# neonbjb/tortoise-tts

Hardware: NVIDIA H100
Metric: audio-seconds/sec at preset='standard' (higher is better)
Workload: dtype bf16 tensor-core operands, fp32 accumulate/residual/norm/softmax/scheduler

## Files before the change

tortoise_tts_b200/csrc/flash_attn.cu:

```cuda
#include <type_traits>

#include "common.cuh"
#include "ttb_internal.h"

namespace ttb {

constexpr int FA_BM = 128;
constexpr int FA_BN = 64;
constexpr int FA_CONSUMERS = 256;
constexpr int FA_PRODUCER_WARP = 8;
constexpr int FA_THREADS = FA_CONSUMERS + 32;
constexpr int FA_STAGES = 2;

struct FaSmem {
  static constexpr int Q_BYTES = FA_BM * 64 * 2;
  static constexpr int K_BYTES = FA_BN * 64 * 2;
  static constexpr int V_BYTES = FA_BN * 64 * 2;
  static constexpr int Q_OFF = 0;
  static constexpr int KV_OFF = Q_BYTES;
  static constexpr int BIAS_OFF = KV_OFF + FA_STAGES * (K_BYTES + V_BYTES);
  static constexpr int BAR_OFF = BIAS_OFF + 192 * 4;
  static constexpr int TOTAL = BAR_OFF + 16 * 8 + 1024;
};

__global__ void __launch_bounds__(FA_THREADS, 2)
flash_attn_tc_kernel(const __grid_constant__ CUtensorMap map_q, const __grid_constant__ CUtensorMap map_k,
                     const __grid_constant__ CUtensorMap map_v, TtbAttnArgs a) {
  extern __shared__ uint8_t smem_raw[];
  uint8_t* smem = reinterpret_cast<uint8_t*>((reinterpret_cast<uintptr_t>(smem_raw) + 1023) & ~uintptr_t(1023));
  uint64_t* bars = reinterpret_cast<uint64_t*>(smem + FaSmem::BAR_OFF);
  uint64_t* q_full = bars + 0;
  uint64_t* kv_full = bars + 1;
  uint64_t* kv_empty = bars + 1 + FA_STAGES;
  float* sbias = reinterpret_cast<float*>(smem + FaSmem::BIAS_OFF);

  const int warp = threadIdx.x >> 5, lane = threadIdx.x & 31;
  const int q0 = blockIdx.x * FA_BM, h = blockIdx.y, seq = blockIdx.z;
  const int Tq = a.T;
  const int T = a.Tk > 0 ? a.Tk : a.T;
  const int kv_end = a.causal ? min(T, q0 + FA_BM) : T;
  const int kc0 = a.kv_headmajor ? 0 : a.k_off + h * 64;
  const int vc0 = a.kv_headmajor ? 0 : a.v_off + h * 64;
  const int kvc2 = a.kv_headmajor ? h : seq;
  const int ntiles = (kv_end + FA_BN - 1) / FA_BN;

  if (warp == FA_PRODUCER_WARP && lane == 0) {
    tma_prefetch_desc(&map_q);
    tma_prefetch_desc(&map_k);
    tma_prefetch_desc(&map_v);
    mbar_init(q_full, 1);
    for (int s = 0; s < FA_STAGES; ++s) { mbar_init(&kv_full[s], 1); mbar_init(&kv_empty[s], 2); }
    fence_barrier_init();
  }
  __syncthreads();
  pdl_wait();

  if (warp == FA_PRODUCER_WARP) {
    if (lane == 0) {
      mbar_arrive_expect_tx(q_full, FaSmem::Q_BYTES);
      tma_load_3d(smem + FaSmem::Q_OFF, &map_q, q_full, h * 64, q0, seq);
      int stage = 0; uint32_t phase = 0;
      for (int j = 0; j < ntiles; ++j) {
        mbar_wait(&kv_empty[stage], phase ^ 1);
        uint8_t* sk = smem + FaSmem::KV_OFF + stage * (FaSmem::K_BYTES + FaSmem::V_BYTES);
        uint8_t* sv = sk + FaSmem::K_BYTES;
        mbar_arrive_expect_tx(&kv_full[stage], FaSmem::K_BYTES + FaSmem::V_BYTES);
        tma_load_3d(sk, &map_k, &kv_full[stage], kc0, j * FA_BN, kvc2);
        tma_load_3d(sv, &map_v, &kv_full[stage], vc0, j * FA_BN, kvc2);
        if (++stage == FA_STAGES) { stage = 0; phase ^= 1; }
      }
    }
    __syncwarp();
  } else {
    const int wg = warp >> 2;
    const int g = lane >> 2, t = lane & 3;
    const int row0 = wg * 64 + (warp & 3) * 16 + g;
    const float sl2 = a.scale * 1.4426950408889634f;
    const float* bias_h = a.bias ? a.bias + (long long)h * (2 * T - 1) + (T - 1) : nullptr;
    float m[2] = {-INFINITY, -INFINITY}, l[2] = {0.f, 0.f};
    float o[32];
#pragma unroll
    for (int i = 0; i < 32; ++i) o[i] = 0.f;
    const uint32_t sq = smem_u32(smem + FaSmem::Q_OFF) + wg * (64 * 128);
    mbar_wait(q_full, 0);
    int stage = 0; uint32_t phase = 0;
    for (int j = 0; j < ntiles; ++j) {
      const int k0 = j * FA_BN;
      const bool nomask = (k0 + FA_BN <= T) && (!a.causal || k0 + FA_BN - 1 <= q0);
      bool cbias_ok = (bias_h == nullptr);
      float cb = 0.f;
      if (bias_h && a.bias_sat > 0) {
        if (k0 - q0 + (FA_BN - 1) <= -a.bias_sat) { cbias_ok = true; cb = __ldg(bias_h - (T - 1)) * 1.4426950408889634f; }
        else if (k0 - q0 - (FA_BM - 1) >= a.bias_sat) { cbias_ok = true; cb = __ldg(bias_h + (T - 1)) * 1.4426950408889634f; }
      }
      const bool fast = nomask && cbias_ok;
      if (bias_h && !fast) {
        named_barrier(1, FA_CONSUMERS);
        for (int i = threadIdx.x; i < 191; i += FA_CONSUMERS) {
          const int rel = k0 - q0 - 127 + i;
          sbias[i] = (rel > -T && rel < T) ? __ldg(bias_h + rel) * 1.4426950408889634f : 0.f;
        }
        named_barrier(1, FA_CONSUMERS);
      }
      mbar_wait(&kv_full[stage], phase);
      const uint32_t sk = smem_u32(smem + FaSmem::KV_OFF + stage * (FaSmem::K_BYTES + FaSmem::V_BYTES));
      const uint32_t sv = sk + FaSmem::K_BYTES;
      float s[32];
      wgmma_fence();
#pragma unroll
      for (int k = 0; k < 4; ++k)
        wgmma_m64n64k16_bf16_ss(s, wgmma_desc_kmajor_sw128(sq + k * 32), wgmma_desc_kmajor_sw128(sk + k * 32), k != 0);
      wgmma_commit();
      wgmma_wait<0>();
      float mx[2] = {-INFINITY, -INFINITY};
      if (fast) {
#pragma unroll
        for (int i = 0; i < 32; ++i) mx[(i >> 1) & 1] = fmaxf(mx[(i >> 1) & 1], s[i]);
        mx[0] = fmaf(mx[0], sl2, cb);
        mx[1] = fmaf(mx[1], sl2, cb);
      } else {
#pragma unroll
        for (int i = 0; i < 32; ++i) {
          const int hh = (i >> 1) & 1;
          const int row = row0 + 8 * hh;
          const int c = 8 * (i >> 2) + 2 * t + (i & 1);
          const int klim = min(T - k0, a.causal ? (q0 + row - k0 + 1) : FA_BN);
          float v = s[i] * sl2;
          if (bias_h) v += sbias[c - row + 127];
          v = (c < klim) ? v : -INFINITY;
          s[i] = v;
          mx[hh] = fmaxf(mx[hh], v);
        }
      }
      float corr[2], cm[2];
#pragma unroll
      for (int hh = 0; hh < 2; ++hh) {
        mx[hh] = fmaxf(mx[hh], __shfl_xor_sync(0xffffffffu, mx[hh], 1));
        mx[hh] = fmaxf(mx[hh], __shfl_xor_sync(0xffffffffu, mx[hh], 2));
        const bool grow = mx[hh] > m[hh] + 8.0f;
        const float m_new = grow ? mx[hh] : m[hh];
        corr[hh] = grow ? exp2f(m[hh] - m_new) : 1.0f;
        m[hh] = m_new;
        const float m_use = (m_new == -INFINITY) ? 0.f : m_new;
        cm[hh] = fast ? cb - m_use : -m_use;
      }
      float psum[2] = {0.f, 0.f};
      uint32_t pa[16];
#pragma unroll
      for (int i = 0; i < 32; i += 2) {
        const int hh = (i >> 1) & 1;
        const float p0 = fast ? exp2f(fmaf(s[i], sl2, cm[hh])) : exp2f(s[i] + cm[hh]);
        const float p1 = fast ? exp2f(fmaf(s[i + 1], sl2, cm[hh])) : exp2f(s[i + 1] + cm[hh]);
        psum[hh] += p0 + p1;
        pa[i >> 1] = pack_bf16(p0, p1);
      }
#pragma unroll
      for (int hh = 0; hh < 2; ++hh) l[hh] = l[hh] * corr[hh] + psum[hh];
#pragma unroll
      for (int i = 0; i < 32; ++i) o[i] *= corr[(i >> 1) & 1];
      wgmma_fence();
#pragma unroll
      for (int k = 0; k < 4; ++k)
        wgmma_m64n64k16_bf16_rs<1>(o, pa + 4 * k, wgmma_desc_mnmajor_sw128(sv + k * 2048, 0), 1u);
      wgmma_commit();
      wgmma_wait<0>();
      if ((threadIdx.x & 127) == 0) mbar_arrive(&kv_empty[stage]);
      if (++stage == FA_STAGES) { stage = 0; phase ^= 1; }
    }
#pragma unroll
    for (int hh = 0; hh < 2; ++hh) {
      l[hh] += __shfl_xor_sync(0xffffffffu, l[hh], 1);
      l[hh] += __shfl_xor_sync(0xffffffffu, l[hh], 2);
      const int qi = q0 + row0 + 8 * hh;
      if (qi >= Tq) continue;
      const float inv = 1.0f / l[hh];
      if (a.lse) {
        float* op = a.out_f32 + ((long long)seq * Tq + qi) * a.ldo + h * 64 + 2 * t;
#pragma unroll
        for (int nb = 0; nb < 8; ++nb)
          *reinterpret_cast<float2*>(op + 8 * nb) = make_float2(o[4 * nb + 2 * hh] * inv, o[4 * nb + 2 * hh + 1] * inv);
        if (t == 0) a.lse[((long long)seq * Tq + qi) * a.H + h] = m[hh] + log2f(l[hh]);
      } else {
        __nv_bfloat16* op = reinterpret_cast<__nv_bfloat16*>(a.out) + ((long long)seq * Tq + qi) * a.ldo + h * 64 + 2 * t;
#pragma unroll
        for (int nb = 0; nb < 8; ++nb)
          *reinterpret_cast<uint32_t*>(op + 8 * nb) = pack_bf16(o[4 * nb + 2 * hh] * inv, o[4 * nb + 2 * hh + 1] * inv);
      }
    }
  }
  pdl_launch_dependents();
}

static int g_fa_mode = -1;

bool flash_attention_supported(const TtbAttnArgs& a) {
  if (g_fa_mode < 0) {
    const char* e = getenv("TTB_ATTN_IMPL");
    g_fa_mode = (e && strcmp(e, "simt") == 0) ? 0 : 1;
  }
  if (!g_fa_mode) return false;
  if (a.kv || a.lse) return true;
  return a.T >= 64 && (a.ld % 8) == 0;
}

int flash_attention_launch(const TtbAttnArgs& a, cudaStream_t st) {
  CUtensorMap mq, mk, mv;
  if (get_tensor_map_bf16(&mq, a.qkv, (uint64_t)a.ld, (uint64_t)a.T, (uint64_t)a.nseq, (uint64_t)a.ld,
                          (uint64_t)a.T * a.ld, 64, FA_BM)) return -1;
  if (a.kv_headmajor) {
    if (!a.kv || !a.kv_v || a.Tk <= 0 || a.causal || a.bias) { set_error("flash attention: bad head-major KV arguments"); return -1; }
    if (get_tensor_map_bf16(&mk, a.kv, 64, (uint64_t)a.Tk, (uint64_t)a.H, 64, (uint64_t)a.Tk * 64, 64, FA_BN)) return -1;
    if (get_tensor_map_bf16(&mv, a.kv_v, 64, (uint64_t)a.Tk, (uint64_t)a.H, 64, (uint64_t)a.Tk * 64, 64, FA_BN)) return -1;
  } else {
    if (a.Tk > 0 && a.Tk != a.T) { set_error("flash attention: Tk != T needs the head-major KV form"); return -1; }
    if (get_tensor_map_bf16(&mk, a.qkv, (uint64_t)a.ld, (uint64_t)a.T, (uint64_t)a.nseq, (uint64_t)a.ld,
                            (uint64_t)a.T * a.ld, 64, FA_BN)) return -1;
    mv = mk;
  }
  if (a.lse && !a.out_f32) { set_error("flash attention: lse output needs out_f32"); return -1; }
  static bool attr = false;
  if (!attr) {
    cudaError_t r = cudaFuncSetAttribute(flash_attn_tc_kernel, cudaFuncAttributeMaxDynamicSharedMemorySize, FaSmem::TOTAL);
    if (r != cudaSuccess) return check_cuda(r, "cudaFuncSetAttribute(flash_attn)");
    attr = true;
  }
  dim3 grid((a.T + FA_BM - 1) / FA_BM, a.H, a.nseq);
  const cudaError_t le = launch_pdl(flash_attn_tc_kernel, grid, dim3(FA_THREADS), (size_t)FaSmem::TOTAL, st, mq, mk, mv, a);
  if (le != cudaSuccess) return check_cuda(le, "flash_attn_tc_kernel launch");
  TTB_CHECK_LAUNCH("flash_attn_tc_kernel");
  return 0;
}

}
```

Baseline: 7.400.

## Make flash attention persistent and warp-specialized with overlapped QK and PV wgmma

Result: faster. 7.492 (median of 6 runs) (+1.2%).

```diff
diff --git a/tortoise_tts_b200/csrc/flash_attn.cu b/tortoise_tts_b200/csrc/flash_attn.cu
--- a/tortoise_tts_b200/csrc/flash_attn.cu
+++ b/tortoise_tts_b200/csrc/flash_attn.cu
@@ -7,184 +7,299 @@
 
 constexpr int FA_BM = 128;
 constexpr int FA_BN = 64;
-constexpr int FA_CONSUMERS = 256;
-constexpr int FA_PRODUCER_WARP = 8;
-constexpr int FA_THREADS = FA_CONSUMERS + 32;
-constexpr int FA_STAGES = 2;
+constexpr int FA_THREADS = 384;
+constexpr int FA_STAGES = 4;
+constexpr int FA_TAB = 1024;
+constexpr float FA_L2E = 1.4426950408889634f;
 
 struct FaSmem {
   static constexpr int Q_BYTES = FA_BM * 64 * 2;
   static constexpr int K_BYTES = FA_BN * 64 * 2;
   static constexpr int V_BYTES = FA_BN * 64 * 2;
+  static constexpr int KV_BYTES = K_BYTES + V_BYTES;
   static constexpr int Q_OFF = 0;
-  static constexpr int KV_OFF = Q_BYTES;
-  static constexpr int BIAS_OFF = KV_OFF + FA_STAGES * (K_BYTES + V_BYTES);
-  static constexpr int BAR_OFF = BIAS_OFF + 192 * 4;
+  static constexpr int KV_OFF = 2 * Q_BYTES;
+  static constexpr int BIAS_OFF = KV_OFF + FA_STAGES * KV_BYTES;
+  static constexpr int BAR_OFF = BIAS_OFF + 2 * FA_TAB * 4;
   static constexpr int TOTAL = BAR_OFF + 16 * 8 + 1024;
 };
 
-__global__ void __launch_bounds__(FA_THREADS, 2)
-flash_attn_tc_kernel(const __grid_constant__ CUtensorMap map_q, const __grid_constant__ CUtensorMap map_k,
+template <int N>
+TTB_DEVINL void fa_pin(float* r) {
+#pragma unroll
+  for (int i = 0; i < N; ++i) asm volatile("" : "+f"(r[i])::"memory");
+}
+template <int N>
+TTB_DEVINL void fa_pin(uint32_t* r) {
+#pragma unroll
+  for (int i = 0; i < N; ++i) asm volatile("" : "+r"(r[i])::"memory");
+}
+
+TTB_DEVINL void fa_unit(const TtbAttnArgs& a, int u, int nqb, int& seq, int& h, int& q0) {
+  const int sh = a.H * a.nseq;
+  const int qb = u / sh, r = u - qb * sh;
+  q0 = (a.causal ? nqb - 1 - qb : qb) * FA_BM;
+  seq = r / a.H;
+  h = r - seq * a.H;
+}
+
+__global__ void __launch_bounds__(FA_THREADS, 1)
+flash_attn_ws_kernel(const __grid_constant__ CUtensorMap map_q, const __grid_constant__ CUtensorMap map_k,
                      const __grid_constant__ CUtensorMap map_v, TtbAttnArgs a) {
   extern __shared__ uint8_t smem_raw[];
   uint8_t* smem = reinterpret_cast<uint8_t*>((reinterpret_cast<uintptr_t>(smem_raw) + 1023) & ~uintptr_t(1023));
   uint64_t* bars = reinterpret_cast<uint64_t*>(smem + FaSmem::BAR_OFF);
   uint64_t* q_full = bars + 0;
-  uint64_t* kv_full = bars + 1;
-  uint64_t* kv_empty = bars + 1 + FA_STAGES;
-  float* sbias = reinterpret_cast<float*>(smem + FaSmem::BIAS_OFF);
+  uint64_t* q_empty = bars + 2;
+  uint64_t* kv_full = bars + 4;
+  uint64_t* kv_empty = bars + 4 + FA_STAGES;
 
   const int warp = threadIdx.x >> 5, lane = threadIdx.x & 31;
-  const int q0 = blockIdx.x * FA_BM, h = blockIdx.y, seq = blockIdx.z;
   const int Tq = a.T;
   const int T = a.Tk > 0 ? a.Tk : a.T;
-  const int kv_end = a.causal ? min(T, q0 + FA_BM) : T;
-  const int kc0 = a.kv_headmajor ? 0 : a.k_off + h * 64;
-  const int vc0 = a.kv_headmajor ? 0 : a.v_off + h * 64;
-  const int kvc2 = a.kv_headmajor ? h : seq;
-  const int ntiles = (kv_end + FA_BN - 1) / FA_BN;
-
-  if (warp == FA_PRODUCER_WARP && lane == 0) {
+  const int nqb = (Tq + FA_BM - 1) / FA_BM;
+  const int units = nqb * a.H * a.nseq;
+
+  if (threadIdx.x == 0) {
     tma_prefetch_desc(&map_q);
     tma_prefetch_desc(&map_k);
     tma_prefetch_desc(&map_v);
-    mbar_init(q_full, 1);
+    for (int b = 0; b < 2; ++b) { mbar_init(&q_full[b], 1); mbar_init(&q_empty[b], 8); }
     for (int s = 0; s < FA_STAGES; ++s) { mbar_init(&kv_full[s], 1); mbar_init(&kv_empty[s], 2); }
     fence_barrier_init();
   }
   __syncthreads();
   pdl_wait();
 
-  if (warp == FA_PRODUCER_WARP) {
-    if (lane == 0) {
-      mbar_arrive_expect_tx(q_full, FaSmem::Q_BYTES);
-      tma_load_3d(smem + FaSmem::Q_OFF, &map_q, q_full, h * 64, q0, seq);
+  if (warp < 4) {
+    setmaxnreg_dec<40>();
+    if (threadIdx.x == 0) {
       int stage = 0; uint32_t phase = 0;
-      for (int j = 0; j < ntiles; ++j) {
-        mbar_wait(&kv_empty[stage], phase ^ 1);
-        uint8_t* sk = smem + FaSmem::KV_OFF + stage * (FaSmem::K_BYTES + FaSmem::V_BYTES);
-        uint8_t* sv = sk + FaSmem::K_BYTES;
-        mbar_arrive_expect_tx(&kv_full[stage], FaSmem::K_BYTES + FaSmem::V_BYTES);
-        tma_load_3d(sk, &map_k, &kv_full[stage], kc0, j * FA_BN, kvc2);
-        tma_load_3d(sv, &map_v, &kv_full[stage], vc0, j * FA_BN, kvc2);
-        if (++stage == FA_STAGES) { stage = 0; phase ^= 1; }
+      int it = 0;
+      for (int u = blockIdx.x; u < units; u += gridDim.x, ++it) {
+        int seq, h, q0;
+        fa_unit(a, u, nqb, seq, h, q0);
+        const int kc0 = a.kv_headmajor ? 0 : a.k_off + h * 64;
+        const int vc0 = a.kv_headmajor ? 0 : a.v_off + h * 64;
+        const int kvc2 = a.kv_headmajor ? h : seq;
+        const int kv_end = a.causal ? min(T, q0 + FA_BM) : T;
+        const int ntiles = (kv_end + FA_BN - 1) / FA_BN;
+        const int qbuf = it & 1;
+        mbar_wait(&q_empty[qbuf], ((it >> 1) & 1) ^ 1);
+        mbar_arrive_expect_tx(&q_full[qbuf], FaSmem::Q_BYTES);
+        tma_load_3d(smem + FaSmem::Q_OFF + qbuf * FaSmem::Q_BYTES, &map_q, &q_full[qbuf], h * 64, q0, seq);
+        for (int j = 0; j < ntiles; ++j) {
+          mbar_wait(&kv_empty[stage], phase ^ 1);
+          uint8_t* sk = smem + FaSmem::KV_OFF + stage * FaSmem::KV_BYTES;
+          mbar_arrive_expect_tx(&kv_full[stage], FaSmem::KV_BYTES);
+          tma_load_3d(sk, &map_k, &kv_full[stage], kc0, j * FA_BN, kvc2);
+          tma_load_3d(sk + FaSmem::K_BYTES, &map_v, &kv_full[stage], vc0, j * FA_BN, kvc2);
+          if (++stage == FA_STAGES) { stage = 0; phase ^= 1; }
+        }
       }
     }
     __syncwarp();
   } else {
-    const int wg = warp >> 2;
+    setmaxnreg_inc<232>();
+    const int wg = (warp >> 2) - 1;
+    const int wtid = threadIdx.x & 127;
     const int g = lane >> 2, t = lane & 3;
     const int row0 = wg * 64 + (warp & 3) * 16 + g;
-    const float sl2 = a.scale * 1.4426950408889634f;
-    const float* bias_h = a.bias ? a.bias + (long long)h * (2 * T - 1) + (T - 1) : nullptr;
-    float m[2] = {-INFINITY, -INFINITY}, l[2] = {0.f, 0.f};
-    float o[32];
-#pragma unroll
-    for (int i = 0; i < 32; ++i) o[i] = 0.f;
-    const uint32_t sq = smem_u32(smem + FaSmem::Q_OFF) + wg * (64 * 128);
-    mbar_wait(q_full, 0);
+    const float sl2 = a.scale * FA_L2E;
+    const int bar_tab = 1 + wg;
+    const bool unit_tab = a.bias && a.bias_sat > 0 && 2 * a.bias_sat + 1 <= FA_TAB;
+    float* tab = reinterpret_cast<float*>(smem + FaSmem::BIAS_OFF) + wg * FA_TAB;
     int stage = 0; uint32_t phase = 0;
-    for (int j = 0; j < ntiles; ++j) {
-      const int k0 = j * FA_BN;
-      const bool nomask = (k0 + FA_BN <= T) && (!a.causal || k0 + FA_BN - 1 <= q0);
-      bool cbias_ok = (bias_h == nullptr);
-      float cb = 0.f;
+    int it = 0;
+    for (int u = blockIdx.x; u < units; u += gridDim.x, ++it) {
+      int seq, h, q0;
+      fa_unit(a, u, nqb, seq, h, q0);
+      const int kv_end = a.causal ? min(T, q0 + FA_BM) : T;
+      const int ntiles = (kv_end + FA_BN - 1) / FA_BN;
+      const float* bias_h = a.bias ? a.bias + (long long)h * (2 * T - 1) + (T - 1) : nullptr;
+      float cb_lo = 0.f, cb_hi = 0.f;
       if (bias_h && a.bias_sat > 0) {
-        if (k0 - q0 + (FA_BN - 1) <= -a.bias_sat) { cbias_ok = true; cb = __ldg(bias_h - (T - 1)) * 1.4426950408889634f; }
-        else if (k0 - q0 - (FA_BM - 1) >= a.bias_sat) { cbias_ok = true; cb = __ldg(bias_h + (T - 1)) * 1.4426950408889634f; }
-      }
-      const bool fast = nomask && cbias_ok;
-      if (bias_h && !fast) {
-        named_barrier(1, FA_CONSUMERS);
-        for (int i = threadIdx.x; i < 191; i += FA_CONSUMERS) {
-          const int rel = k0 - q0 - 127 + i;
-          sbias[i] = (rel > -T && rel < T) ? __ldg(bias_h + rel) * 1.4426950408889634f : 0.f;
-        }
-        named_barrier(1, FA_CONSUMERS);
-      }
+        cb_lo = __ldg(bias_h - (T - 1)) * FA_L2E;
+        cb_hi = __ldg(bias_h + (T - 1)) * FA_L2E;
+      }
+      if (unit_tab) {
+        named_barrier(bar_tab, 128);
+        for (int i = wtid; i <= 2 * a.bias_sat; i += 128) {
+          const int rel = i - a.bias_sat;
+          tab[i] = (rel > -T && rel < T) ? __ldg(bias_h + rel) * FA_L2E : 0.f;
+        }
+        named_barrier(bar_tab, 128);
+      }
+      const int qbuf = it & 1;
+      mbar_wait(&q_full[qbuf], (it >> 1) & 1);
+      uint32_t qa[16];
+      {
+        const uint8_t* sq = smem + FaSmem::Q_OFF + qbuf * FaSmem::Q_BYTES;
+        const int r = row0;
+#pragma unroll
+        for (int k = 0; k < 4; ++k) {
+#pragma unroll
+          for (int hi = 0; hi < 2; ++hi) {
+            const int chunk = (2 * k + hi) ^ (r & 7);
+            qa[4 * k + 2 * hi] = *reinterpret_cast<const uint32_t*>(sq + r * 128 + chunk * 16 + 4 * t);
+            qa[4 * k + 2 * hi + 1] = *reinterpret_cast<const uint32_t*>(sq + (r + 8) * 128 + chunk * 16 + 4 * t);
+          }
+        }
+      }
+      __syncwarp();
+      if (lane == 0) mbar_arrive(&q_empty[qbuf]);
+
+      float m[2] = {-INFINITY, -INFINITY}, l[2] = {0.f, 0.f};
+      float o[32], s[32], corr[2];
+      float x[32];
+      uint32_t pa[16];
+#pragma unroll
+      for (int i = 0; i < 32; ++i) o[i] = 0.f;
+
+      auto issue_s = [&](int st) {
+        const uint32_t sk = smem_u32(smem + FaSmem::KV_OFF + st * FaSmem::KV_BYTES);
+#pragma unroll
+        for (int k = 0; k < 4; ++k) wgmma_m64n64k16_bf16_rs<0>(s, qa + 4 * k, wgmma_desc_kmajor_sw128(sk + k * 32), k != 0);
+        wgmma_commit();
+      };
+      auto issue_pv = [&](int st) {
+        const uint32_t sv = smem_u32(smem + FaSmem::KV_OFF + st * FaSmem::KV_BYTES + FaSmem::K_BYTES);
+#pragma unroll
+        for (int k = 0; k < 4; ++k) wgmma_m64n64k16_bf16_rs<1>(o, pa + 4 * k, wgmma_desc_mnmajor_sw128(sv + k * 2048, 0), 1u);
+        wgmma_commit();
+      };
+      auto softmax = [&](int j) {
+        const int k0 = j * FA_BN;
+        const bool nomask = (k0 + FA_BN <= T) && (!a.causal || k0 + FA_BN - 1 <= q0);
+        bool cbias_ok = (bias_h == nullptr);
+        float cb = 0.f;
+        if (bias_h && a.bias_sat > 0) {
+          if (k0 - q0 + (FA_BN - 1) <= -a.bias_sat) { cbias_ok = true; cb = cb_lo; }
+          else if (k0 - q0 - (FA_BM - 1) >= a.bias_sat) { cbias_ok = true; cb = cb_hi; }
+        }
+        const bool fast = nomask && cbias_ok;
+        int lo = -a.bias_sat, hi = a.bias_sat;
+        if (bias_h && !fast && !unit_tab) {
+          lo = k0 - q0 - wg * 64 - 63;
+          hi = lo + 126;
+          named_barrier(bar_tab, 128);
+          for (int i = wtid; i < 127; i += 128) {
+            const int rel = lo + i;
+            tab[i] = (rel > -T && rel < T) ? __ldg(bias_h + rel) * FA_L2E : 0.f;
+          }
+          named_barrier(bar_tab, 128);
+        }
+        float mx[2] = {-INFINITY, -INFINITY};
+        if (fast) {
+#pragma unroll
+          for (int i = 0; i < 32; ++i) {
+            x[i] = s[i];
+            mx[(i >> 1) & 1] = fmaxf(mx[(i >> 1) & 1], s[i]);
+          }
+          mx[0] = fmaf(mx[0], sl2, cb);
+          mx[1] = fmaf(mx[1], sl2, cb);
+        } else {
+#pragma unroll
+          for (int i = 0; i < 32; ++i) {
+            const int hh = (i >> 1) & 1;
+            const int row = row0 + 8 * hh;
+            const int c = 8 * (i >> 2) + 2 * t + (i & 1);
+            const int klim = min(T - k0, a.causal ? (q0 + row - k0 + 1) : FA_BN);
+            float v = s[i] * sl2;
+            if (bias_h) v += tab[min(max(k0 + c - q0 - row, lo), hi) - lo];
+            v = (c < klim) ? v : -INFINITY;
+            x[i] = v;
+            mx[hh] = fmaxf(mx[hh], v);
+          }
+        }
+        float cm[2];
+#pragma unroll
+        for (int hh = 0; hh < 2; ++hh) {
+          mx[hh] = fmaxf(mx[hh], __shfl_xor_sync(0xffffffffu, mx[hh], 1));
+          mx[hh] = fmaxf(mx[hh], __shfl_xor_sync(0xffffffffu, mx[hh], 2));
+          const bool grow = mx[hh] > m[hh] + 8.0f;
+          const float m_new = grow ? mx[hh] : m[hh];
+          corr[hh] = grow ? exp2f(m[hh] - m_new) : 1.0f;
+          m[hh] = m_new;
+          const float m_use = (m_new == -INFINITY) ? 0.f : m_new;
+          cm[hh] = fast ? cb - m_use : -m_use;
+        }
+        float psum[2] = {0.f, 0.f};
+#pragma unroll
+        for (int i = 0; i < 32; i += 2) {
+          const int hh = (i >> 1) & 1;
+          const float p0 = exp2f(fast ? fmaf(x[i], sl2, cm[hh]) : x[i] + cm[hh]);
+          const float p1 = exp2f(fast ? fmaf(x[i + 1], sl2, cm[hh]) : x[i + 1] + cm[hh]);
+          psum[hh] += p0 + p1;
+          x[i] = p0;
+          x[i + 1] = p1;
+        }
+#pragma unroll
+        for (int hh = 0; hh < 2; ++hh) l[hh] = l[hh] * corr[hh] + psum[hh];
+        fa_pin<32>(x);
+        fa_pin<2>(corr);
+        fa_pin<2>(l);
+      };
+      auto rescale_and_pack = [&]() {
+#pragma unroll
+        for (int i = 0; i < 32; ++i) o[i] *= corr[(i >> 1) & 1];
+#pragma unroll
+        for (int i = 0; i < 32; i += 2) pa[i >> 1] = pack_bf16(x[i], x[i + 1]);
+        fa_pin<16>(pa);
+        fa_pin<32>(o);
+      };
+      auto release = [&](int st) { if (wtid == 0) mbar_arrive(&kv_empty[st]); };
+
       mbar_wait(&kv_full[stage], phase);
-      const uint32_t sk = smem_u32(smem + FaSmem::KV_OFF + stage * (FaSmem::K_BYTES + FaSmem::V_BYTES));
-      const uint32_t sv = sk + FaSmem::K_BYTES;
-      float s[32];
       wgmma_fence();
-#pragma unroll
-      for (int k = 0; k < 4; ++k)
-        wgmma_m64n64k16_bf16_ss(s, wgmma_desc_kmajor_sw128(sq + k * 32), wgmma_desc_kmajor_sw128(sk + k * 32), k != 0);
-      wgmma_commit();
+      issue_s(stage);
       wgmma_wait<0>();
-      float mx[2] = {-INFINITY, -INFINITY};
-      if (fast) {
-#pragma unroll
-        for (int i = 0; i < 32; ++i) mx[(i >> 1) & 1] = fmaxf(mx[(i >> 1) & 1], s[i]);
-        mx[0] = fmaf(mx[0], sl2, cb);
-        mx[1] = fmaf(mx[1], sl2, cb);
-      } else {
-#pragma unroll
-        for (int i = 0; i < 32; ++i) {
-          const int hh = (i >> 1) & 1;
-          const int row = row0 + 8 * hh;
-          const int c = 8 * (i >> 2) + 2 * t + (i & 1);
-          const int klim = min(T - k0, a.causal ? (q0 + row - k0 + 1) : FA_BN);
-          float v = s[i] * sl2;
-          if (bias_h) v += sbias[c - row + 127];
-          v = (c < klim) ? v : -INFINITY;
-          s[i] = v;
-          mx[hh] = fmaxf(mx[hh], v);
-        }
-      }
-      float corr[2], cm[2];
+      fa_pin<32>(s);
+      softmax(0);
+      rescale_and_pack();
+      int prev = stage;
+      if (++stage == FA_STAGES) { stage = 0; phase ^= 1; }
+      for (int j = 1; j < ntiles; ++j) {
+        mbar_wait(&kv_full[stage], phase);
+          wgmma_fence();
+        issue_s(stage);
+        issue_pv(prev);
+          wgmma_wait<1>();
+        fa_pin<32>(s);
+        softmax(j);
+        wgmma_wait<0>();
+        fa_pin<32>(o);
+        fa_pin<16>(pa);
+        release(prev);
+        rescale_and_pack();
+        prev = stage;
+        if (++stage == FA_STAGES) { stage = 0; phase ^= 1; }
+      }
+      wgmma_fence();
+      issue_pv(prev);
+      wgmma_wait<0>();
+      fa_pin<32>(o);
+      fa_pin<16>(pa);
+      release(prev);
 #pragma unroll
       for (int hh = 0; hh < 2; ++hh) {
-        mx[hh] = fmaxf(mx[hh], __shfl_xor_sync(0xffffffffu, mx[hh], 1));
-        mx[hh] = fmaxf(mx[hh], __shfl_xor_sync(0xffffffffu, mx[hh], 2));
-        const bool grow = mx[hh] > m[hh] + 8.0f;
-        const float m_new = grow ? mx[hh] : m[hh];
-        corr[hh] = grow ? exp2f(m[hh] - m_new) : 1.0f;
-        m[hh] = m_new;
-        const float m_use = (m_new == -INFINITY) ? 0.f : m_new;
-        cm[hh] = fast ? cb - m_use : -m_use;
-      }
-      float psum[2] = {0.f, 0.f};
-      uint32_t pa[16];
-#pragma unroll
-      for (int i = 0; i < 32; i += 2) {
-        const int hh = (i >> 1) & 1;
-        const float p0 = fast ? exp2f(fmaf(s[i], sl2, cm[hh])) : exp2f(s[i] + cm[hh]);
-        const float p1 = fast ? exp2f(fmaf(s[i + 1], sl2, cm[hh])) : exp2f(s[i + 1] + cm[hh]);
-        psum[hh] += p0 + p1;
-        pa[i >> 1] = pack_bf16(p0, p1);
-      }
-#pragma unroll
-      for (int hh = 0; hh < 2; ++hh) l[hh] = l[hh] * corr[hh] + psum[hh];
-#pragma unroll
-      for (int i = 0; i < 32; ++i) o[i] *= corr[(i >> 1) & 1];
-      wgmma_fence();
-#pragma unroll
-      for (int k = 0; k < 4; ++k)
-        wgmma_m64n64k16_bf16_rs<1>(o, pa + 4 * k, wgmma_desc_mnmajor_sw128(sv + k * 2048, 0), 1u);
-      wgmma_commit();
-      wgmma_wait<0>();
-      if ((threadIdx.x & 127) == 0) mbar_arrive(&kv_empty[stage]);
-      if (++stage == FA_STAGES) { stage = 0; phase ^= 1; }
-    }
-#pragma unroll
-    for (int hh = 0; hh < 2; ++hh) {
-      l[hh] += __shfl_xor_sync(0xffffffffu, l[hh], 1);
-      l[hh] += __shfl_xor_sync(0xffffffffu, l[hh], 2);
-      const int qi = q0 + row0 + 8 * hh;
-      if (qi >= Tq) continue;
-      const float inv = 1.0f / l[hh];
-      if (a.lse) {
-        float* op = a.out_f32 + ((long long)seq * Tq + qi) * a.ldo + h * 64 + 2 * t;
-#pragma unroll
-        for (int nb = 0; nb < 8; ++nb)
-          *reinterpret_cast<float2*>(op + 8 * nb) = make_float2(o[4 * nb + 2 * hh] * inv, o[4 * nb + 2 * hh + 1] * inv);
-        if (t == 0) a.lse[((long long)seq * Tq + qi) * a.H + h] = m[hh] + log2f(l[hh]);
-      } else {
-        __nv_bfloat16* op = reinterpret_cast<__nv_bfloat16*>(a.out) + ((long long)seq * Tq + qi) * a.ldo + h * 64 + 2 * t;
-#pragma unroll
-        for (int nb = 0; nb < 8; ++nb)
-          *reinterpret_cast<uint32_t*>(op + 8 * nb) = pack_bf16(o[4 * nb + 2 * hh] * inv, o[4 * nb + 2 * hh + 1] * inv);
+        l[hh] += __shfl_xor_sync(0xffffffffu, l[hh], 1);
+        l[hh] += __shfl_xor_sync(0xffffffffu, l[hh], 2);
+        const int qi = q0 + row0 + 8 * hh;
+        if (qi >= Tq) continue;
+        const float inv = 1.0f / l[hh];
+        if (a.lse) {
+          float* op = a.out_f32 + ((long long)seq * Tq + qi) * a.ldo + h * 64 + 2 * t;
+#pragma unroll
+          for (int nb = 0; nb < 8; ++nb)
+            *reinterpret_cast<float2*>(op + 8 * nb) = make_float2(o[4 * nb + 2 * hh] * inv, o[4 * nb + 2 * hh + 1] * inv);
+          if (t == 0) a.lse[((long long)seq * Tq + qi) * a.H + h] = m[hh] + log2f(l[hh]);
+        } else {
+          __nv_bfloat16* op = reinterpret_cast<__nv_bfloat16*>(a.out) + ((long long)seq * Tq + qi) * a.ldo + h * 64 + 2 * t;
+#pragma unroll
+          for (int nb = 0; nb < 8; ++nb)
+            *reinterpret_cast<uint32_t*>(op + 8 * nb) = pack_bf16(o[4 * nb + 2 * hh] * inv, o[4 * nb + 2 * hh + 1] * inv);
+        }
       }
     }
   }
@@ -219,15 +334,21 @@
   }
   if (a.lse && !a.out_f32) { set_error("flash attention: lse output needs out_f32"); return -1; }
   static bool attr = false;
+  static int num_sms = 0;
   if (!attr) {
-    cudaError_t r = cudaFuncSetAttribute(flash_attn_tc_kernel, cudaFuncAttributeMaxDynamicSharedMemorySize, FaSmem::TOTAL);
+    cudaError_t r = cudaFuncSetAttribute(flash_attn_ws_kernel, cudaFuncAttributeMaxDynamicSharedMemorySize, FaSmem::TOTAL);
     if (r != cudaSuccess) return check_cuda(r, "cudaFuncSetAttribute(flash_attn)");
+    int dev = 0;
+    r = cudaGetDevice(&dev);
+    if (r == cudaSuccess) r = cudaDeviceGetAttribute(&num_sms, cudaDevAttrMultiProcessorCount, dev);
+    if (r != cudaSuccess) return check_cuda(r, "flash attention: SM count");
     attr = true;
   }
-  dim3 grid((a.T + FA_BM - 1) / FA_BM, a.H, a.nseq);
-  const cudaError_t le = launch_pdl(flash_attn_tc_kernel, grid, dim3(FA_THREADS), (size_t)FaSmem::TOTAL, st, mq, mk, mv, a);
-  if (le != cudaSuccess) return check_cuda(le, "flash_attn_tc_kernel launch");
-  TTB_CHECK_LAUNCH("flash_attn_tc_kernel");
+  const long long units = (long long)((a.T + FA_BM - 1) / FA_BM) * a.H * a.nseq;
+  const dim3 grid((unsigned)(units < num_sms ? units : num_sms));
+  const cudaError_t le = launch_pdl(flash_attn_ws_kernel, grid, dim3(FA_THREADS), (size_t)FaSmem::TOTAL, st, mq, mk, mv, a);
+  if (le != cudaSuccess) return check_cuda(le, "flash_attn_ws_kernel launch");
+  TTB_CHECK_LAUNCH("flash_attn_ws_kernel");
   return 0;
 }
 
```
